# JinPLu/VeloxSeg

Hardware: AMD Instinct MI355X
Metric: training patches/s on 128^3 2-mod volumes (fwd+loss+bwd+allreduce+AdamW) (higher is better)
Workload: dtype f32

## Files before the change

### include/veloxseg_hip.h

```cpp
#ifndef VELOXSEG_HIP_H
#define VELOXSEG_HIP_H

#ifdef __cplusplus
extern "C" {
#endif

#define VX_ABI_VERSION 1

int vx_abi_version(void);
const char* vx_last_error(void);

int vx_conv3d_fwd(const float* x, const float* x2, int C1, const float* w, const float* bias, float* y,
                  int B, int Cin, int Di, int Hi, int Wi, int Cout, int K, int S, int P, int G, int ps, void* stream);
int vx_conv3d_bwd_data(const float* dy, const float* w, const float* bias_like, float* dx, float* dx2, int C1,
                       int B, int Cin, int Di, int Hi, int Wi, int Cout, int K, int S, int P, int G, int ps,
                       int accumulate, void* stream);
int vx_conv3d_bwd_weight(const float* x, const float* x2, int C1, const float* dy, float* dw, float* db,
                         int B, int Cin, int Di, int Hi, int Wi, int Cout, int K, int S, int P, int G, int ps, void* stream);

int vx_conv3d_bwd_weight_tiled(const float* x, const float* x2, int C1, const float* dy, float* dw, float* db,
                               int B, int Cin, int Di, int Hi, int Wi, int Cout, int K, int S, int P, int G, int ps, void* stream);
int vx_down_wgrad_ws_floats(int B, int Cin, int Di, int Hi, int Wi, int Cout);
int vx_down_wgrad_mfma(const float* x, const float* dy, float* dw, float* db, float* ws, long ws_floats,
                       int B, int Cin, int Di, int Hi, int Wi, int Cout, void* stream);
// ... 32 lines not shown
                   int B, int Cin, int Cout, long V, void* stream);
int vx_pw_conv_set_v4(int on);
int vx_pw_conv_bwd_data(const float* dy, const float* w, float* dx, float* dx2, int C1,
                        int B, int Cin, int Cout, long V, int accumulate, void* stream);
int vx_pw_conv_bwd_weight(const float* x, const float* x2, int C1, const float* dy, float* dw, float* db,
                          int B, int Cin, int Cout, long V, void* stream);
int vx_pw_conv_fwd_h(const void* x, const float* w, const float* bias, float* y, int B, int Cin, int Cout, long V, int x_h16, void* stream);
int vx_pw_conv_bwd_weight_h(const void* x, const float* dy, float* dw, float* db, int B, int Cin, int Cout, long V, int x_h16, void* stream);

int vx_pw_conv_mfma(const float* src, const float* src2, int S1, const float* w, int transpose_w, const float* bias,
                    float* dst, float* dst2, int D1, int B, int Mch, int Kch, int Cin_of_w, long V, int accumulate, void* stream);
int vx_pw_conv_bwd_fused(const float* dy, const float* w, const float* x, const float* x2, int C1, float* dx, float* dx2, float* dw, float* db,
                         int B, int Cin, int Cout, long V, int accumulate, void* stream);
int vx_pw_conv_bwd_fused_big(const float* dy, const float* w, const float* x, const float* x2, int C1, float* dx, float* dx2, float* dw, float* db,
                             int B, int Cin, int Cout, long V, int accumulate, void* stream);
int vx_pw_conv_gelu_fwd(const float* x, const float* w, const float* bias, float* a, float* h, int B, int Cin, int Cout, long V, int mfma,
                        const void* seed_ptr, unsigned long long dstream, float p, void* stream);
int vx_pw_conv_gelu_bwd_data(const float* dy, const float* w, const float* a, float* da, int B, int Cin, int Cout, long V, int mfma,
                             const void* seed_ptr, unsigned long long dstream, float p, void* stream);
int vx_pw_conv_res_fwd(const float* x, const float* w, const float* bias, const float* res, float* out, int B, int Cin, int Cout, long V, int mfma,
                       float alpha, const void* seed_ptr, unsigned long long dstream, float p, void* stream);
int vx_pw_mfma_set_wide(int on);

int vx_mlp_supported(int C, int R, long V);
int vx_mlp_bwd_nparts(int B, int C, long V);
int vx_mlp_fwd(const float* x, int norm, const double* part, int nparts, float* stats, const float* gamma, const float* beta,
               const float* w1, const float* b1, const float* w2, const float* b2, float* out, int B, int C, int R, long V, float eps,
               const void* seed_ptr, unsigned long long site1, float p1, unsigned long long site2, float p2, void* stream);
int vx_mlp_bwd(const float* x, int norm, const float* stats, const float* gamma, const float* beta, const float* w1, const float* b1,
               const float* w2, const float* dout, float* dx, float* part_out, float* dgamma, float* dbeta, float* dw1, float* db1,
               float* dw2, float* db2, int B, int C, int R, long V, float eps, const void* seed_ptr, unsigned long long site1, float p1,
               unsigned long long site2, float p2, void* stream);
int vx_jlc_ntiles(int B, int C, int G, int D, int H, int W);
int vx_jlc_nchunks(long BC, long V);
int vx_jlc_conv_fwd(const float* x, const float* w1, const float* w3, const float* w5, const float* b1, const float* b3, const float* b5,
                    float* y1, float* y3, float* y5, double* part, int B, int C, int G, int D, int H, int W, void* stream);
int vx_jlc_mid_fwd(const float* x, const float* y1, const float* y3, const float* y5, const double* part_y, int nty, float* stats_y, float* o,
                   double* part_o, long BC, long V, float eps, void* stream);
int vx_jlc_mid_bwd(const float* dout, const float* dn, const float* part_dn, int npd, const float* o, const float* stats_o, const float* y1,
                   const float* y3, const float* y5, const float* stats_y, float* d_o, float* part_t, long BC, long V, void* stream);
int vx_jlc_gk(const float* d_o, const float* y1, const float* y3, const float* y5, const float* stats_y, const float* part_t, float* g1, float* g3,
              float* g5, long BC, long V, void* stream);
int vx_jlc_conv_bwd(const float* g1, const float* g3, const float* g5, const float* w1, const float* w3, const float* w5, const float* d_o,
                    float* dx, int B, int C, int G, int D, int H, int W, void* stream);
int vx_jlc_mid_fwd_h(const float* x, const void* y1, const void* y3, const void* y5, const double* part_y, int nty, float* stats_y, void* o,
                     double* part_o, long BC, long V, float eps, int h16, void* stream);
int vx_jlc_mid_bwd_h(const float* dout, const void* dn, const float* part_dn, int npd, const void* o, const float* stats_o, const void* y1,
                     const void* y3, const void* y5, const float* stats_y, void* d_o, float* part_t, long BC, long V, int h16, void* stream);
int vx_jlc_gk_h(const void* d_o, const void* y1, const void* y3, const void* y5, const float* stats_y, const float* part_t, void* g1, void* g3,
                void* g5, long BC, long V, int h16, void* stream);
int vx_mlp_fwd_h(const void* x, int norm, const double* part, int nparts, float* stats, const float* gamma, const float* beta,
                 const float* w1, const float* b1, const float* w2, const float* b2, float* out, int B, int C, int R, long V, float eps,
                 const void* seed_ptr, unsigned long long site1, float p1, unsigned long long site2, float p2, int h16, void* stream);
int vx_mlp_bwd_h(const void* x, int norm, const float* stats, const float* gamma, const float* beta, const float* w1, const float* b1,
                 const float* w2, const float* dout, void* dx, float* part_out, float* dgamma, float* dbeta, float* dw1, float* db1,
                 float* dw2, float* db2, int B, int C, int R, long V, float eps, const void* seed_ptr, unsigned long long site1, float p1,
                 unsigned long long site2, float p2, int h16, void* stream);

int vx_jlc_tz_ok(int C, int G, int D, int H, int W);
int vx_jlc_tz_ntiles(int C, int G, int D, int H, int W);
int vx_jlc_tz_img_floats(int C, int G);
int vx_jlc_tz_set_pieces(int ns);
int vx_jlc_tz_set_min_voxels(long v);
int vx_jlc_tz_pieces(void);
int vx_jlc_tz_set_debug(int mask);
int vx_jlc_tz_prep(const float* w1, const float* w3, const float* w5, float* img, int C, int G, void* stream);
int vx_jlc_tz_fwd(const float* x, const float* img, const float* b1, const float* b3, const float* b5, float* y1, float* y3, float* y5, double* part,
                  int B, int C, int G, int D, int H, int W, void* stream);
int vx_jlc_tz_bwd(const float* g1, const float* g3, const float* g5, const float* img, const float* w1, const float* d_o, float* dx,
                  int B, int C, int G, int D, int H, int W, void* stream);
int vx_jlc_cl_ok(int C, int G, int D, int H, int W);
int vx_jlc_cl_ntiles(int C, int G, int D, int H, int W);
int vx_jlc_cl_img_floats(int C, int G);
int vx_jlc_cl_set_enabled(int on);
int vx_jlc_cl_prep(const float* w1, const float* w3, const float* w5, float* img, int C, int G, void* stream);
int vx_jlc_cl_fwd(const float* x, const float* img, const float* b1, const float* b3, const float* b5, float* y1, float* y3, float* y5, double* part,
                  int B, int C, int G, int D, int H, int W, void* stream);
int vx_jlc_cl_bwd(const float* g1, const float* g3, const float* g5, const float* img, const float* d_o, float* dx, int B, int C, int G, int D, int H, int W,
                  void* stream);
int vx_jlc_wgrad_tz_ok(int C, int G, int D, int H, int W);
int vx_jlc_wgrad_tz_set_min_voxels(long v);
int vx_jlc_wgrad_tz_set_blocks(int n);
int vx_jlc_wgrad_tz_set_spec(int on);
int vx_jlc_wgrad_tz_set_f16(int on);
int vx_jlc_wgrad_tz(const float* x, const float* g1, const float* g3, const float* g5, float* dw1, float* dw3, float* dw5, int B, int C, int G, int D, int H, int W,
                    void* stream);
int vx_jlc_tz_img_floats_ns(int C, int G, int pieces);
int vx_jlc_tz_prep_ns(const float* w1, const float* w3, const float* w5, float* img, int C, int G, int pieces, void* stream);
int vx_jlc_tz_fwd_ns(const float* x, const float* img, const float* b1, const float* b3, const float* b5, float* y1, float* y3, float* y5, double* part,
                     int B, int C, int G, int D, int H, int W, int pieces, void* stream);
int vx_jlc_tz_bwd_ns(const float* g1, const float* g3, const float* g5, const float* img, const float* w1, const float* d_o, float* dx,
                     int B, int C, int G, int D, int H, int W, int pieces, void* stream);
int vx_jlc_wgrad_tz_ns(const float* x, const float* g1, const float* g3, const float* g5, float* dw1, float* dw3, float* dw5, int B, int C, int G, int D, int H, int W,
                       int pieces, void* stream);
int vx_jlc_tz_fwd_h(const float* x, const float* img, const float* b1, const float* b3, const float* b5, void* y1, void* y3, void* y5, double* part,
                    int B, int C, int G, int D, int H, int W, int pieces, int h16, void* stream);
int vx_jlc_tz_bwd_h(const void* g1, const void* g3, const void* g5, const float* img, const float* w1, const void* d_o, float* dx,
                    int B, int C, int G, int D, int H, int W, int pieces, int h16, void* stream);
int vx_jlc_wgrad_tz_h(const float* x, const void* g1, const void* g3, const void* g5, float* dw1, float* dw3, float* dw5, int B, int C, int G, int D, int H, int W,
                      int pieces, int h16, void* stream);

int vx_in_stats(const float* x, float* stats, double* part_ws, long BC, long V, float eps, void* stream);
int vx_in_apply_fwd(const float* y0, const float* y1, const float* y2, const float* s0, const float* s1, const float* s2,
                    int nk, int act, const float* res, float* out, long BC, long V, void* stream);
int vx_in_bwd(const float* dout, const float* y, const float* stats, int act, float* m_ws, double* part_ws, float* dy, long BC, long V, void* stream);
int vx_in_row_max(void);
int vx_in_row_fwd(const float* y0, const float* y1, const float* y2, float* s0, float* s1, float* s2, int nk, int act, const float* res,
                  float* out, long BC, long V, float eps, void* stream);
int vx_in_row_bwd(const float* dout, const float* y0, const float* y1, const float* y2, const float* s0, const float* s1, const float* s2,
                  int nk, int act, float* d0, float* d1, float* d2, long BC, long V, void* stream);
int vx_in_bwd_db(const float* dout, const float* y, const float* stats, int act, float* m_ws, double* part_ws, float* dy, long BC, long V, float* db, int C, void* stream);
int vx_in_fwd_split(const float* y0, const float* y1, const float* y2, float* s0, float* s1, float* s2, double* part_ws,
                    int nk, int act, const float* res, float* out, long BC, long V, float eps, void* stream);
int vx_in_bwd_split(const float* dout, const float* y0, const float* y1, const float* y2, const float* s0, const float* s1, const float* s2,
                    double* part_ws, int nk, int act, float* dy0, float* dy1, float* dy2, const float* add0, long BC, long V, void* stream);
int vx_in_row_bwd_add(const float* dout, const float* y0, const float* stats0, int act, const float* add0, float* d0, long BC, long V, void* stream);
int vx_in_row_bwd_db(const float* dout, const float* y0, const float* y1, const float* y2, const float* s0, const float* s1, const float* s2,
                     int nk, int act, float* d0, float* d1, float* d2, float* db0, float* db1, float* db2, int C, long BC, long V, void* stream);

int vx_ln_cf_fwd(const float* x, const float* gamma, const float* beta, float* out, int B, int C, long V, float eps, void* stream);
int vx_ln_cf_bwd(const float* x, const float* gamma, const float* dout, float* dx, float* dgamma, float* dbeta, float* ws,
                 int B, int C, long V, float eps, void* stream);
int vx_ln_cf_bwd_add(const float* x, const float* gamma, const float* dout, const float* add, float* dx, float* dgamma, float* dbeta, float* ws,
                     int B, int C, long V, float eps, void* stream);
int vx_ln_cf_bwd_data(const float* x, const float* gamma, const float* dout, const float* add, float* dx, float* ws, int B, int C, long V, float eps, void* stream);
int vx_ln_cf_bwd_param(const float* x, const float* dout, const float* ws, float* dgamma, float* dbeta, int B, int C, long V, void* stream);

int vx_gelu_drop_fwd(const float* a, float* h, long n, const void* seed_ptr, unsigned long long dstream, float p, void* stream);
int vx_gelu_drop_bwd(const float* dh, const float* a, float* da, long n, const void* seed_ptr, unsigned long long dstream, float p, void* stream);
int vx_axpy_drop_fwd(const float* x, const float* z, float* out, float alpha, long n, const void* seed_ptr, unsigned long long dstream, float p, void* stream);
int vx_axpy_drop_bwd(const float* dout, float* dx, float* dz, float alpha, long n, const void* seed_ptr, unsigned long long dstream, float p, void* stream);
int vx_add(const float* a, const float* b, const float* c, float* out, long n, void* stream);
int vx_add_many(const float* const* a, const float* const* b, const float* const* c, float* const* out, const long* n, int count, void* stream);
int vx_channel_sum(const float* dy, float* db, int B, int C, long V, void* stream);
int vx_space_to_depth2(const float* x, float* out, int B, int C, int Dc, int Hc, int Wc, int inverse, void* stream);
int vx_patchify(const float* x, float* out, int B, int C, int d, int h, int w, int K, void* stream);
int vx_patchify_bs(const float* x, long batch_stride, float* out, int B, int C, int d, int h, int w, int K, void* stream);
int vx_patchify_bs_h(const float* x, long batch_stride, void* out, int B, int C, int d, int h, int w, int K, int out_h16, void* stream);
int vx_patch_embed_ok(int Cin, int Cout, int Do, int Ho, int Wo, int K);
int vx_patch_embed_fwd(const float* x, long batch_stride, const float* w, const float* bias, float* y, int B, int Cin, int Cout, int Do, int Ho, int Wo, void* stream);
int vx_patch_embed_bwd_weight(const float* x, long batch_stride, const float* dy, float* dw, float* db, int B, int Cin, int Cout, int Do, int Ho, int Wo, void* stream);

typedef struct VxPwaPlan {
    int grid[3];
    int n[3];
    int heads, nb;
    int small[4][3];
    int nwin[4][3];
    int woff[4];
    int Ntot;
    int l;
} VxPwaPlan;

int vx_pwa_gather_fwd(const float* src, float* tok, const VxPwaPlan* plan, int c, int m, int M, int B, void* stream);
int vx_pwa_gather_bwd(const float* src, const float* dtok, float* dsrc, const VxPwaPlan* plan, int c, int m, int M, int B, void* stream);
int vx_pwa_gather_all_fwd(const float* const* srcs, float* tq, float* tk, float* tv, int* iq, int* ik, int* iv,
                          const VxPwaPlan* plan, int cq, int cv, int M, int B, void* stream);
int vx_pwa_gather_all_bwd(const float* dtq, const float* dtk, const float* dtv, const int* iq, const int* ik, const int* iv, float* const* dsrcs,
                          const VxPwaPlan* plan, int cq, int cv, int M, int B, void* stream);
int vx_pwa_scatter_fwd(const float* tok, float* out, const VxPwaPlan* plan, int c, int m, int M, int B, void* stream);
int vx_pwa_scatter_bwd(const float* dout, float* dtok, const VxPwaPlan* plan, int c, int m, int M, int B, void* stream);
int vx_pwa_scatter_fwd_all(const float* tok, float* const* outs, const VxPwaPlan* plan, int c, int M, int B, void* stream);
int vx_pwa_scatter_bwd_all(const float* const* douts, float* dtok, const VxPwaPlan* plan, int c, int M, int B, void* stream);
int vx_pwa_scatter_bwd_all_w(const float* const* douts, float* dtok, const VxPwaPlan* plan, int c, int M, int B, void* stream);
int vx_pwa_scatter_bwd_all_wz(const float* const* douts, float* dtok, const VxPwaPlan* plan, int c, int M, int B, float* extra_zero, long extra_floats, void* stream);
int vx_pwa_attn_set_fused_bwd(int on);
int vx_pwa_scatter_set_ident(int on);
// ... 174 lines not shown
```

### veloxseg_amd/csrc/jlc_mfma.hip

```cpp
#include "vx_common.h"
#include <type_traits>
#include "../../include/veloxseg_hip.h"

typedef __bf16 tz_bf8 __attribute__((ext_vector_type(8)));
typedef float tz_f4 __attribute__((ext_vector_type(4)));

struct TzGeo {
    int HD, HH;
    int Sd, Sc, Sp;
    int nrows;
    unsigned mHH, mHD;
    int qd0, nq;
    unsigned mNQ;
};

struct VxTz {
    const void* src[3];
    const uint4* img;
    const float* esc;
    const float* bias[3];
    const void* res;
    const float* w1;
    void* out[3];
    double* part;
// ... 740 lines not shown
        if (s + 1 < NS) { a0 -= tz_lo(lo); a1 -= tz_hi(lo); a2 -= tz_lo(hi); a3 -= tz_hi(hi); }
    }
}

#define WG_NPF 6
struct WgDesc { const char* b; int l, f; };
template <bool H16 = false>
__device__ __forceinline__ WgDesc wg_desc(const VxWgT& p, int it, int sg, int cob, int cib, int h0) {
    WgDesc r;
    r.b = (const char*)p.x; r.l = 0; r.f = 0;
    const int nqx = p.XR / 4, rows = p.TH + 4;
    const int nx = p.nb * 4 * rows * nqx;
    const int chan = p.D * p.H * p.W;
    if (it < nx) {
        const int qd = it % nqx; int t = it / nqx;
        const int row = t % rows; t /= rows;
        const int ci = t & 3, s = t >> 2;
        const int b = sg * p.nb + s, ih = h0 - 2 + row, iw = 4 * qd - 4;
        const bool ok = b < p.B && (unsigned)ih < (unsigned)p.H && (unsigned)iw < (unsigned)p.W;
        r.f = 4 | (ok ? 8 : 0);
        r.b = (const char*)(p.x + (ok ? (long)(b * p.C + cib + ci) * chan + ih * p.W + iw : 0));
        r.l = ((s * 4 + ci) * rows + row) * p.XR + 4 * qd;
        return r;
    }
    it -= nx;
    const int nqg = p.WS / 4;
    const int ng = p.nb * 4 * p.TH * nqg;
    const int kind = it / ng;
    if (kind > 2) return r;
    it -= kind * ng;
    const int qd = it % nqg; int t = it / nqg;
    const int row = t % p.TH; t /= p.TH;
    const int co = t & 3, s = t >> 2;
    const int b = sg * p.nb + s, ih = h0 + row, iw = 4 * qd;
    const bool ok = b < p.B && ih < p.H && iw < p.W;
    r.f = (kind + 1) | 4 | (ok ? 8 : 0);
    r.b = (const char*)(kind == 0 ? p.g5 : kind == 1 ? p.g3 : p.g1) + (H16 ? 2L : 4L) * (ok ? (long)(b * p.C + cob + co) * chan + ih * p.W + iw : 0);
    r.l = p.GB + ((s * 4 + co) * (p.TH + 1) + row) * p.WS + 4 * qd;
    return r;
}
__device__ __forceinline__ int wg_dk(int k) { return (0x18 >> (2 * k)) & 3; }
template <bool SP> __device__ __forceinline__ int wg_s5(const VxWgT&, int pl) { return (pl + 60) % (SP ? 6 : 5); }
template <bool SP> __device__ __forceinline__ int wg_s3(const VxWgT&, int pl) { return (SP ? 6 : 5) + (pl + 60) % (SP ? 4 : 3); }
template <bool SP> __device__ __forceinline__ int wg_s1(const VxWgT&, int pl) { return SP ? 10 + ((pl + 60) & 1) : 8; }
template <bool SP> __device__ __forceinline__ int wg_xo(const VxWgT& p, int dx) { return SP ? ((dx + 60) & 1) * p.XP : 0; }
template <bool H16 = false>
__device__ __forceinline__ void wg_prefetch(float4 (&pf)[WG_NPF], const WgDesc (&ds)[WG_NPF], const VxWgT& p, int dx, int dg0, int dg1) {
    const long HW = (long)p.H * p.W;
#pragma unroll
    for (int u = 0; u < WG_NPF; ++u) {
        const int k = ds[u].f & 3;
        const int pl = dx + wg_dk(k);
        const bool on = (ds[u].f & 8) && pl >= (k == 0 ? 0 : dg0) && pl < (k == 0 ? p.D : dg1);
        typedef const __attribute__((address_space(1))) tz_f4* wg_gptr;
        if constexpr (H16) {
            typedef unsigned int wg_u2 __attribute__((ext_vector_type(2)));
            typedef const __attribute__((address_space(1))) wg_u2* wg_gptr2;
            const bool isx = k == 0;
            const unsigned long long ga = (unsigned long long)ds[u].b + (isx ? 4ull : 2ull) * (unsigned long long)(on ? (long)pl * HW : 0);
            float4 r;
            if (isx) { const tz_f4 v = *(wg_gptr)ga; r = make_float4(v[0], v[1], v[2], v[3]); }
            else { const wg_u2 v = *(wg_gptr2)ga; r = make_float4(vx_bf16_lo(v[0]), vx_bf16_hi(v[0]), vx_bf16_lo(v[1]), vx_bf16_hi(v[1])); }
            pf[u] = on ? r : make_float4(0.f, 0.f, 0.f, 0.f);
        } else {
        const unsigned long long ga = (unsigned long long)ds[u].b + 4ull * (unsigned long long)(on ? (long)pl * HW : 0);
        const tz_f4 v = *(wg_gptr)ga;
        pf[u] = on ? make_float4(v[0], v[1], v[2], v[3]) : make_float4(0.f, 0.f, 0.f, 0.f);
        }
    }
}
template <int NS, bool SP = false>
__device__ __forceinline__ void wg_commit(const float4 (&pf)[WG_NPF], const WgDesc (&ds)[WG_NPF], unsigned char* lds, const VxWgT& p, int dx, int dg0, int dg1) {
    const int l5 = wg_s5<SP>(p, dx + 2) * p.GP, l3 = wg_s3<SP>(p, dx + 1) * p.GP, l1 = wg_s1<SP>(p, dx) * p.GP, lx = wg_xo<SP>(p, dx);
#pragma unroll
    for (int u = 0; u < WG_NPF; ++u) {
        const int k = ds[u].f & 3;
        const int pl = dx + wg_dk(k);
        const bool on = (ds[u].f & 4) && pl >= (k == 0 ? 0 : dg0) && pl < (k == 0 ? p.D : dg1);
        const int lo = k == 0 ? lx : k == 1 ? l5 : k == 2 ? l3 : l1;
        if (on) wg_split_store<NS>(pf[u], lds, (long)ds[u].l + lo, p.SP);
    }
}

__device__ __forceinline__ void wg_commit16(const float4 (&pf)[WG_NPF], const WgDesc (&ds)[WG_NPF], unsigned char* lds, const VxWgT& p, int dx, int dg0, int dg1,
                                            float* __restrict__ mtab, int* __restrict__ etab) {
    const int s5 = wg_s5<false>(p, dx + 2), s3 = wg_s3<false>(p, dx + 1), s1_ = wg_s1<false>(p, dx);
    const int l5 = s5 * p.GP, l3 = s3 * p.GP, l1 = s1_ * p.GP;
    float mk[4] = {0.f, 0.f, 0.f, 0.f};
    bool on_[WG_NPF];
#pragma unroll
    for (int u = 0; u < WG_NPF; ++u) {
        const int k = ds[u].f & 3;
        const int pl = dx + wg_dk(k);
        on_[u] = (ds[u].f & 4) && pl >= (k == 0 ? 0 : dg0) && pl < (k == 0 ? p.D : dg1);
        const float m_ = on_[u] ? fmaxf(fmaxf(fabsf(pf[u].x), fabsf(pf[u].y)), fmaxf(fabsf(pf[u].z), fabsf(pf[u].w))) : 0.0f;
#pragma unroll
        for (int kk = 0; kk < 4; ++kk) mk[kk] = fmaxf(mk[kk], k == kk ? m_ : 0.0f);
    }
#pragma unroll
    for (int kk = 0; kk < 4; ++kk) mk[kk] = vx_wave_max(mk[kk]);
    if ((threadIdx.x & 63) == 0) {
#pragma unroll
        for (int kk = 0; kk < 4; ++kk) mtab[(threadIdx.x >> 6) * 4 + kk] = mk[kk];
    }
    __syncthreads();
    int ek[4];
#pragma unroll
    for (int kk = 0; kk < 4; ++kk) ek[kk] = tz_exp16(fmaxf(fmaxf(mtab[kk], mtab[4 + kk]), fmaxf(mtab[8 + kk], mtab[12 + kk])));
    if (threadIdx.x == 0) {
        etab[0] = ek[0];
        etab[1 + s5] = ek[1]; etab[1 + s3] = ek[2]; etab[1 + s1_] = ek[3];
    }
#pragma unroll
    for (int u = 0; u < WG_NPF; ++u) {
        if (!on_[u]) continue;
        const int k = ds[u].f & 3;
        const int lo = k == 0 ? 0 : k == 1 ? l5 : k == 2 ? l3 : l1;
        const float sc = ldexpf(1.0f, k == 0 ? ek[0] : k == 1 ? ek[1] : k == 2 ? ek[2] : ek[3]);
        const float a0 = pf[u].x * sc, a1 = pf[u].y * sc, a2 = pf[u].z * sc, a3 = pf[u].w * sc;
        const uint32_t lo0 = tz_pack16(a0, a1), hi0 = tz_pack16(a2, a3);
        const uint32_t lo1 = tz_pack16(a0 - tz_lo16(lo0), a1 - tz_hi16(lo0)), hi1 = tz_pack16(a2 - tz_lo16(hi0), a3 - tz_hi16(hi0));
        const long e0 = (long)ds[u].l + lo;
        *reinterpret_cast<uint2*>(lds + 2 * e0) = make_uint2(lo0, hi0);
        *reinterpret_cast<uint2*>(lds + 2 * ((long)p.SP + e0)) = make_uint2(lo1, hi1);
    }
}

template <int NS>
__device__ __forceinline__ void wg_read_a(uint4 (&a)[NS], const unsigned char* lds, const VxWgT& p, int slot, int arow_base, int local, int th_lane) {
    const int j = threadIdx.x & 3;
    const int r = local + j;
    const int rr = (unsigned)r < (unsigned)th_lane ? r : p.TH;
#pragma unroll
    for (int s = 0; s < NS; ++s)
        a[s] = *reinterpret_cast<const uint4*>(lds + 2 * ((long)s * p.SP + p.GB + (long)slot * p.GP + (long)arow_base + (long)rr * p.WS));
}

template <int NS, bool F16 = false>
__device__ __forceinline__ void wg_mfma6(tz_f4& acc, const uint4 (&a)[NS], const uint4 (&b)[NS]) {
    constexpr int NP = NS == 3 ? 6 : NS == 2 ? 3 : 1;
    constexpr int PW[6] = {1, 2, 0, 1, 0, 0}, PA[6] = {1, 0, 2, 0, 1, 0};
    constexpr int PW2[3] = {1, 0, 0}, PA2[3] = {0, 1, 0};
#pragma unroll
    for (int pr = 0; pr < NP; ++pr) {
        const int sa = NS == 3 ? PW[pr] : NS == 2 ? PW2[pr] : 0, sb = NS == 3 ? PA[pr] : NS == 2 ? PA2[pr] : 0;
        if constexpr (F16) acc = __builtin_amdgcn_mfma_f32_16x16x32_f16(__builtin_bit_cast(tz_h8, a[sa]), __builtin_bit_cast(tz_h8, b[sb]), acc, 0, 0, 0);
        else acc = __builtin_amdgcn_mfma_f32_16x16x32_bf16(__builtin_bit_cast(tz_bf8, a[sa]), __builtin_bit_cast(tz_bf8, b[sb]), acc, 0, 0, 0);
    }
}

__device__ __forceinline__ uint4 wg_shift(const uint32_t (&w)[8], int o) {
    const int d = o >> 1;
    if ((o & 1) == 0) return make_uint4(w[d], w[d + 1], w[d + 2], w[d + 3]);
    return make_uint4(__builtin_amdgcn_alignbit(w[d + 1], w[d], 16), __builtin_amdgcn_alignbit(w[d + 2], w[d + 1], 16), __builtin_amdgcn_alignbit(w[d + 3], w[d + 2], 16),
                      __builtin_amdgcn_alignbit(w[d + 4], w[d + 3], 16));
}

template <int NS, bool DBG, bool F16 = false, bool SPEC = false, bool H16 = false>
__global__ void __launch_bounds__(SPEC ? 512 : 256, SPEC ? 1 : 2) vx_jlc_wg_k(VxWgT p_) {
    const VxWgT& p = p_;
    const int dbg = DBG ? p_.dbg : 0;
    extern __shared__ __attribute__((aligned(16))) unsigned char wg_lds[];
    const int lane = threadIdx.x & 63;
    const int wave = __builtin_amdgcn_readfirstlane((int)(threadIdx.x >> 6));
    const int r16 = lane & 15, q = lane >> 4;
    int bid = blockIdx.x;
    const int dc = bid % p.nDc; bid /= p.nDc;
    const int ht = bid % p.nHt; bid /= p.nHt;
    const int MT = p.CG >> 2;
    const int ih = bid % MT; bid /= MT;
    const int ch = bid % MT; bid /= MT;
    const int g = bid % p.G;
    const int sg = bid / p.G;
    const int h0 = ht * p.TH;
    const int dg0 = dc * p.DC, dg1 = min(p.D, dg0 + p.DC);
    const int cob = g * p.CG + ch * 4, cib = g * p.CG + ih * 4;

    constexpr int nslot = SPEC ? 12 : 9;
    for (int it = threadIdx.x; it < nslot * p.nb * 4 * (p.WS / 2) * NS; it += blockDim.x) {
        int r = it;
        const int e2 = r % (p.WS / 2); r /= (p.WS / 2);
        const int sc = r % (p.nb * 4); r /= (p.nb * 4);
        const int slot = r % nslot, s = r / nslot;
        *reinterpret_cast<uint32_t*>(wg_lds + 2 * ((long)s * p.SP + p.GB + (long)slot * p.GP + ((long)sc * (p.TH + 1) + p.TH) * p.WS + 2 * e2)) = 0u;
    }
    const int smp_ = (8 * q) / p.WS;
    const bool nosmp = smp_ >= p.nb;
    const int smp = nosmp ? 0 : smp_, wq = nosmp ? 0 : 8 * q - smp_ * p.WS;
    const int arow_base = ((smp * 4 + (r16 >> 2)) * (p.TH + 1)) * p.WS + wq;
    const int brow_base = ((smp * 4 + (r16 >> 2)) * (p.TH + 4) + (r16 & 3)) * p.XR + wq;
    const int th_lane = nosmp ? 0 : p.TH;

    tz_f4 acc[20];
    float* mtab = reinterpret_cast<float*>(wg_lds + 2 * (long)NS * p.SP);
    int* etab = reinterpret_cast<int*>(mtab + 16);
    int ecur[5] = {0, 0, 0, 0, 0};
    const bool producer = SPEC && wave >= 4;
    if (SPEC && producer) {
        float4 pf[WG_NPF];
        WgDesc ds[WG_NPF];
#pragma unroll
        for (int u = 0; u < WG_NPF; ++u) ds[u] = wg_desc<H16>(p, (int)(threadIdx.x & 255) + u * 256, sg, cob, cib, h0);
        wg_prefetch<H16>(pf, ds, p, dg0 - 2, dg0, dg1);
        __syncthreads();
        wg_commit<NS, true>(pf, ds, wg_lds, p, dg0 - 2, dg0, dg1);
        wg_prefetch<H16>(pf, ds, p, dg0 - 1, dg0, dg1);
        __syncthreads();
        for (int dx = dg0 - 2; dx <= dg1 + 1; ++dx) {
            if (dx + 1 <= dg1 + 1) {
                wg_commit<NS, true>(pf, ds, wg_lds, p, dx + 1, dg0, dg1);
                if (dx + 2 <= dg1 + 1) wg_prefetch<H16>(pf, ds, p, dx + 2, dg0, dg1);
            }
            __syncthreads();
        }
    } else {
#pragma unroll
    for (int t = 0; t < 20; ++t) acc[t] = (tz_f4){0.f, 0.f, 0.f, 0.f};
    float4 pf[WG_NPF];
    WgDesc ds[WG_NPF];
    if constexpr (!SPEC) {
#pragma unroll
        for (int u = 0; u < WG_NPF; ++u) ds[u] = wg_desc<H16>(p, (int)threadIdx.x + u * 256, sg, cob, cib, h0);
        wg_prefetch<H16>(pf, ds, p, dg0 - 2, dg0, dg1);
    } else {
        __syncthreads();
        __syncthreads();
    }
    for (int dx = dg0 - 2; dx <= dg1 + 1; ++dx) {
        if constexpr (SPEC) {
            if ((unsigned)dx >= (unsigned)p.D) { __syncthreads(); continue; }
        } else {
        __syncthreads();
        if constexpr (F16) wg_commit16(pf, ds, wg_lds, p, dx, dg0, dg1, mtab, etab);
        else if (!(dbg & 1)) wg_commit<NS>(pf, ds, wg_lds, p, dx, dg0, dg1);
        __syncthreads();
        if (dx + 1 <= dg1 + 1 && !(dbg & 1)) wg_prefetch<H16>(pf, ds, p, dx + 1, dg0, dg1);
        if (dbg & 2) continue;
        if ((unsigned)dx >= (unsigned)p.D) continue;
        }
        const bool k3w = wave < 3;
        const int kd0 = k3w ? wave : 3, kd1 = k3w ? wave : 4;
        const int pl0 = dx - kd0 + 2, pl1 = k3w ? dx - kd1 + 1 : dx - kd1 + 2;
        const bool ok0 = pl0 >= dg0 && pl0 < dg1, ok1 = pl1 >= dg0 && pl1 < dg1, okc = wave == 0 && dx >= dg0 && dx < dg1;
        const int so0 = wg_s5<SPEC>(p, pl0), so1 = k3w ? wg_s3<SPEC>(p, pl1) : wg_s5<SPEC>(p, pl1);
        const int xo8 = wg_xo<SPEC>(p, dx) >> 3;
        if constexpr (F16) {
            const int e_x = __builtin_amdgcn_readfirstlane(etab[0]);
            auto bring = [&](int which, int slot, int lo, int n_) {
                const int ep = e_x + __builtin_amdgcn_readfirstlane(etab[1 + slot]);
                if (ep == ecur[which]) return;
                const int dd = ep - ecur[which];
                const float f = ldexpf(1.0f, dd > 120 ? 120 : (dd < -120 ? -120 : dd));
#pragma unroll
                for (int t = 0; t < 20; ++t)
                    if (t >= lo && t < lo + n_ && !(which == 1 && k3w && (t == 13 || t == 14 || t == 18 || t == 19))) acc[t] *= f;
                ecur[which] = ep;
            };
            if (ok0) bring(0, so0, 0, 10);
            if (ok1) bring(1, so1, 10, 10);
            if (okc) {
                const int ep = e_x + __builtin_amdgcn_readfirstlane(etab[1 + wg_s1<SPEC>(p, dx)]);
                if (ep != ecur[4]) {
                    const int dd = ep - ecur[4];
                    acc[13] *= ldexpf(1.0f, dd > 120 ? 120 : (dd < -120 ? -120 : dd));
                    ecur[4] = ep;
                }
            }
        }
        for (int xb = 0; xb < p.nXB; ++xb) {
            uint32_t w[NS][8];
#pragma unroll
            for (int s = 0; s < NS; ++s) {
                const int eo = ((s * (p.SP >> 3) + xo8 + (brow_base >> 3) + 4 * xb * (p.XR >> 3)) << 3);
                const uint4* bp = reinterpret_cast<const uint4*>(wg_lds + 2 * (long)eo);
                const uint4 lo = bp[0], hi = bp[1];
                w[s][0] = lo.x; w[s][1] = lo.y; w[s][2] = lo.z; w[s][3] = lo.w; w[s][4] = hi.x; w[s][5] = hi.y; w[s][6] = hi.z; w[s][7] = hi.w;
            }
            uint4 sh[5][NS];
#pragma unroll
            for (int k = 0; k < 5; ++k)
#pragma unroll
                for (int s = 0; s < NS; ++s) sh[k][s] = wg_shift(w[s], k + 2);
            uint4 a[NS];
#pragma unroll
            for (int u = 0; u < 4; ++u) {
                const int sl = u >> 1, typ = u & 1;
                const bool k3 = sl == 1 && k3w;
                if (!(sl ? ok1 : ok0)) continue;
                const int local = 4 * xb - (typ ? 4 : 0) - (k3 ? 1 : 0);
                if (local + 3 < 0 || local >= p.TH) continue;
                if (!(dbg & 16)) wg_read_a<NS>(a, wg_lds, p, sl ? so1 : so0, arow_base, local, th_lane);
#pragma unroll
                for (int k = 0; k < 5; ++k) {
                    if (k >= 3 && k3) continue;
                    if (!(dbg & 8)) wg_mfma6<NS, F16>(acc[5 * u + k], a, sh[sl ? (k + 1) % 5 : k]);
                }
            }
            if (okc) {
                wg_read_a<NS>(a, wg_lds, p, wg_s1<SPEC>(p, dx), arow_base, 4 * xb - 2, th_lane);
                wg_mfma6<NS, F16>(acc[13], a, sh[2]);
            }
        }
        if constexpr (SPEC) __syncthreads();
    }
    }
    if (dbg & 4) return;
    float* tl = reinterpret_cast<float*>(wg_lds);
    if constexpr (F16) {
        const float f0 = ldexpf(1.0f, -ecur[0]), f1 = ldexpf(1.0f, -ecur[1]), f13 = ldexpf(1.0f, -ecur[4]);
#pragma unroll
        for (int t = 0; t < 20; ++t) {
            if (t < 10) acc[t] *= f0;
            else if (wave < 3 && (t == 13 || t == 14 || t == 18 || t == 19)) { if (t == 13) acc[t] *= f13; }
            else acc[t] *= f1;
        }
    }
#pragma unroll
    for (int sl = 0; sl < 2; ++sl) {
        __syncthreads();
        if (!SPEC || wave < 4) {
#pragma unroll
        for (int t = 0; t < 10; ++t)
            *reinterpret_cast<float4*>(tl + (((wave * 10 + t) * 16 + r16) * 16 + 4 * q)) = make_float4(acc[sl * 10 + t][0], acc[sl * 10 + t][1], acc[sl * 10 + t][2], acc[sl * 10 + t][3]);
        }
        __syncthreads();
        const int n5 = sl == 0 ? 1600 : 400, n3 = sl == 0 ? 0 : 432;
        for (int it = threadIdx.x; it < n5 + n3; it += blockDim.x) {
            const bool k3 = it >= n5;
            const int o = k3 ? it - n5 : it;
            const int K = k3 ? 3 : 5, per = k3 ? 27 : (sl == 0 ? 100 : 25);
            const int pair = o / per, r = o - pair * per;
            const int kdl = r / (K * K), r2 = r - kdl * K * K;
            const int kh = r2 / K, kw = r2 - kh * K;
            const int kd = k3 ? kdl : (sl == 0 ? kdl : 4);
            const int wv = k3 ? kd : (kd < 3 ? kd : 3);
            const int co = pair >> 2, ci = pair & 3;
            const int kt = (!k3 && sl == 1) ? (kw + 4) % 5 : kw;
            float v = 0.0f;
#pragma unroll
            for (int typ = 0; typ < 2; ++typ) {
                const float* T = tl + ((wv * 10 + typ * 5 + kt) * 16) * 16;
                const int d = kh - (typ ? 4 : 0);
#pragma unroll
                for (int jj = 0; jj < 4; ++jj) {
                    const int i = jj + d;
                    if (i >= 0 && i < 4) v += T[(ci * 4 + i) * 16 + co * 4 + jj];
                }
            }
            float* dst = k3 ? p.dw3 : p.dw5;
            const int K3 = K * K * K;
            if (dst) atomicAdd(dst + ((long)(cob + co) * p.CG + ih * 4 + ci) * K3 + (kd * K + kh) * K + kw, v);
        }
        if (sl == 1 && p.dw1) {
            for (int pair = threadIdx.x; pair < 16; pair += blockDim.x) {
                const int co = pair >> 2, ci = pair & 3;
                const float* T = tl + ((0 * 10 + 3) * 16) * 16;
                float v = 0.0f;
#pragma unroll
                for (int jj = 0; jj < 4; ++jj) v += T[(ci * 4 + jj) * 16 + co * 4 + jj];
                atomicAdd(p.dw1 + (long)(cob + co) * p.CG + ih * 4 + ci, v);
            }
        }
    }
}

static int g_wg_blocks = 0;
extern "C" int vx_jlc_wgrad_tz_set_blocks(int n) { g_wg_blocks = n > 0 ? n : 0; return 0; }
static int g_wg_spec = 1;
extern "C" int vx_jlc_wgrad_tz_set_spec(int on) { g_wg_spec = on ? 1 : 0; return 0; }
static bool wg_spec_on() { return g_wg_spec == 1; }
static int wg_plan(VxWgT& p, size_t& shm, int B, int C, int G, int D, int H, int W, int NS, bool spec = false) {
    if (B <= 0 || C <= 0 || G <= 0 || C % G || D <= 0 || H <= 0 || W <= 0 || (W & 3) || (H & 3) || W > 32) return -1;
    const int CG = C / G;
    if (CG != 4 && CG != 8 && CG != 16) return -1;
    p.B = B; p.C = C; p.G = G; p.D = D; p.H = H; p.W = W; p.CG = CG;
    p.WS = (W + 7) / 8 * 8;
    p.nb = 32 / p.WS;
    p.nsg = vx_cdiv(B, p.nb);
    p.TH = H % 8 == 0 ? 8 : 4;
    p.nHt = H / p.TH;
    p.nXB = p.TH / 4 + 1;
    p.XR = p.WS + 8;
    p.XP = p.nb * 4 * (p.TH + 4) * p.XR;
    p.GP = p.nb * 4 * (p.TH + 1) * p.WS;
    p.XB = spec ? 2 : 1; p.R5 = spec ? 6 : 5; p.R3 = spec ? 4 : 3; p.R1 = spec ? 2 : 1;
    p.GB = p.XB * p.XP;
    p.SP = p.GB + (p.R5 + p.R3 + p.R1) * p.GP;
    const int MT = CG / 4;
    const long base_blocks = (long)p.nsg * G * MT * MT * p.nHt;
    const int target = g_wg_blocks > 0 ? g_wg_blocks : (spec ? 128 : 256);
    int nchunks = (int)((target + base_blocks - 1) / base_blocks);
    constexpr int min_dc = 2;
    if (nchunks > D / min_dc) nchunks = D / min_dc;
    if (nchunks < 1) nchunks = 1;
    p.DC = vx_cdiv(D, nchunks);
    p.nDc = vx_cdiv(D, p.DC);
    if ((long)p.nb * 4 * (p.TH + 4) * (p.XR / 4) + 3L * p.nb * 4 * p.TH * (p.WS / 4) > (long)WG_NPF * 256) return -1;
    shm = (size_t)NS * p.SP * 2 + 128;
    if (shm < 4 * 10 * 256 * sizeof(float)) shm = 4 * 10 * 256 * sizeof(float);
    if (shm > 150 * 1024) return -1;
    return 0;
}

static long g_wg_min_v = 0;
static int g_wg_f16 = 0;
extern "C" int vx_jlc_wgrad_tz_set_f16(int on) { g_wg_f16 = on ? 1 : 0; return 0; }
extern "C" int vx_jlc_wgrad_tz_set_min_voxels(long v) { g_wg_min_v = v < 0 ? 0 : v; return 0; }
extern "C" int vx_jlc_wgrad_tz_ok(int C, int G, int D, int H, int W) {
    VxWgT p = {};
    size_t shm;
    if ((long)D * H * W < g_wg_min_v) return 0;
    return wg_plan(p, shm, 1, C, G, D, H, W, tz_pieces() == 22 ? 3 : tz_pieces()) == 0 ? 1 : 0;
}

extern "C" int vx_jlc_wgrad_tz(const float* x, const float* g1, const float* g3, const float* g5, float* dw1, float* dw3, float* dw5, int B, int C, int G, int D, int H, int W,
                               void* stream) {
    VX_REQUIRE(x && g1 && g3 && g5, "vx_jlc_wgrad_tz: null pointer");
    VxWgT p = {};
    size_t shm;
    const bool f16 = tz_pieces() == 22 && g_wg_f16 == 1;
    const int NS = f16 ? 2 : (tz_pieces() == 22 ? 3 : tz_pieces());
    VX_REQUIRE(!t_tz_h16 || NS == 1, "vx_jlc_wgrad_tz: 16-bit g_k need plain bf16 operands (pieces = 1, the bf16 mode)");
    bool spec = !f16 && NS == 3 && (g_tz_dbg >> 4) == 0 && wg_spec_on();
    if (spec) { VxWgT q = {}; size_t sh2; spec = wg_plan(q, sh2, B, C, G, D, H, W, NS, true) == 0; }
    VX_REQUIRE(wg_plan(p, shm, B, C, G, D, H, W, NS, spec) == 0, "vx_jlc_wgrad_tz: unsupported shape C=%d G=%d %dx%dx%d", C, G, D, H, W);
    p.x = x; p.g1 = g1; p.g3 = g3; p.g5 = g5; p.dw1 = dw1; p.dw3 = dw3; p.dw5 = dw5; p.dbg = g_tz_dbg >> 4;
    const int MT = p.CG / 4;
    const dim3 grid((unsigned)((long)p.nsg * G * MT * MT * p.nHt * p.nDc));
    hipStream_t st = (hipStream_t)stream;
#define WG_LAUNCH(ns)                                                                                                                                      \
    do {                                                                                                                                                   \
        static bool attr = false;                                                                                                                          \
        if (!attr) {                                                                                                                                       \
            VX_REQUIRE(hipFuncSetAttribute((const void*)vx_jlc_wg_k<ns, false>, hipFuncAttributeMaxDynamicSharedMemorySize, 160 * 1024) == hipSuccess &&           \
                       hipFuncSetAttribute((const void*)vx_jlc_wg_k<ns, true>, hipFuncAttributeMaxDynamicSharedMemorySize, 160 * 1024) == hipSuccess, "vx_jlc_wgrad_tz: LDS attribute"); \
            attr = true;                                                                                                                                   \
        }                                                                                                                                                  \
        if (p.dbg) vx_jlc_wg_k<ns, true><<<grid, dim3(256), shm, st>>>(p);                                                                                 \
        else vx_jlc_wg_k<ns, false><<<grid, dim3(256), shm, st>>>(p);                                                                                      \
    } while (0)
    if (spec) {
        static bool attrs = false;
        if (!attrs) { VX_REQUIRE(hipFuncSetAttribute((const void*)vx_jlc_wg_k<3, false, false, true>, hipFuncAttributeMaxDynamicSharedMemorySize, 160 * 1024) == hipSuccess, "vx_jlc_wgrad_tz: LDS attribute"); attrs = true; }
        vx_jlc_wg_k<3, false, false, true><<<grid, dim3(512), shm, st>>>(p);
    } else if (f16) {
        static bool attr16 = false;
        if (!attr16) { VX_REQUIRE(hipFuncSetAttribute((const void*)vx_jlc_wg_k<2, false, true>, hipFuncAttributeMaxDynamicSharedMemorySize, 160 * 1024) == hipSuccess, "vx_jlc_wgrad_tz: LDS attribute"); attr16 = true; }
        vx_jlc_wg_k<2, false, true><<<grid, dim3(256), shm, st>>>(p);
    } else if (NS == 3) WG_LAUNCH(3); else if (NS == 2) WG_LAUNCH(2);
    else if (t_tz_h16) {
        static bool attrh = false;
        if (!attrh) { VX_REQUIRE(hipFuncSetAttribute((const void*)vx_jlc_wg_k<1, false, false, false, true>, hipFuncAttributeMaxDynamicSharedMemorySize, 160 * 1024) == hipSuccess, "vx_jlc_wgrad_tz: LDS attribute"); attrh = true; }
        vx_jlc_wg_k<1, false, false, false, true><<<grid, dim3(256), shm, st>>>(p);
    } else WG_LAUNCH(1);
#undef WG_LAUNCH
    VX_LAUNCH_CHECK("vx_jlc_wgrad_tz");
    return 0;
}

extern "C" int vx_jlc_tz_img_floats_ns(int C, int G, int pieces) {
    if (!tz_pieces_valid(pieces)) return -1;
    TzPiecesScope sc(pieces);
    return vx_jlc_tz_img_floats(C, G);
}
extern "C" int vx_jlc_tz_prep_ns(const float* w1, const float* w3, const float* w5, float* img, int C, int G, int pieces, void* stream) {
    VX_REQUIRE(tz_pieces_valid(pieces), "vx_jlc_tz_prep_ns: pieces %d", pieces);
    TzPiecesScope sc(pieces);
    return vx_jlc_tz_prep(w1, w3, w5, img, C, G, stream);
}
extern "C" int vx_jlc_tz_fwd_ns(const float* x, const float* img, const float* b1, const float* b3, const float* b5, float* y1, float* y3, float* y5, double* part,
                                int B, int C, int G, int D, int H, int W, int pieces, void* stream) {
    VX_REQUIRE(tz_pieces_valid(pieces), "vx_jlc_tz_fwd_ns: pieces %d", pieces);
    TzPiecesScope sc(pieces);
    return vx_jlc_tz_fwd(x, img, b1, b3, b5, y1, y3, y5, part, B, C, G, D, H, W, stream);
}
extern "C" int vx_jlc_tz_bwd_ns(const float* g1, const float* g3, const float* g5, const float* img, const float* w1, const float* d_o, float* dx,
                                int B, int C, int G, int D, int H, int W, int pieces, void* stream) {
    VX_REQUIRE(tz_pieces_valid(pieces), "vx_jlc_tz_bwd_ns: pieces %d", pieces);
    TzPiecesScope sc(pieces);
    return vx_jlc_tz_bwd(g1, g3, g5, img, w1, d_o, dx, B, C, G, D, H, W, stream);
}
extern "C" int vx_jlc_tz_fwd_h(const float* x, const float* img, const float* b1, const float* b3, const float* b5, void* y1, void* y3, void* y5, double* part,
                               int B, int C, int G, int D, int H, int W, int pieces, int h16, void* stream) {
    VX_REQUIRE(tz_pieces_valid(pieces), "vx_jlc_tz_fwd_h: pieces %d", pieces);
    TzPiecesScope sc(pieces);
    TzH16Scope hs(h16 ? 1 : 0);
    return vx_jlc_tz_fwd(x, img, b1, b3, b5, (float*)y1, (float*)y3, (float*)y5, part, B, C, G, D, H, W, stream);
}
extern "C" int vx_jlc_tz_bwd_h(const void* g1, const void* g3, const void* g5, const float* img, const float* w1, const void* d_o, float* dx,
                               int B, int C, int G, int D, int H, int W, int pieces, int h16, void* stream) {
    VX_REQUIRE(tz_pieces_valid(pieces), "vx_jlc_tz_bwd_h: pieces %d", pieces);
    TzPiecesScope sc(pieces);
    TzH16Scope hs(h16 ? 1 : 0);
    return vx_jlc_tz_bwd((const float*)g1, (const float*)g3, (const float*)g5, img, w1, (const float*)d_o, dx, B, C, G, D, H, W, stream);
}
extern "C" int vx_jlc_wgrad_tz_h(const float* x, const void* g1, const void* g3, const void* g5, float* dw1, float* dw3, float* dw5, int B, int C, int G, int D, int H, int W,
                                 int pieces, int h16, void* stream) {
    VX_REQUIRE(tz_pieces_valid(pieces), "vx_jlc_wgrad_tz_h: pieces %d", pieces);
    TzPiecesScope sc(pieces);
    TzH16Scope hs(h16 ? 1 : 0);
    return vx_jlc_wgrad_tz(x, (const float*)g1, (const float*)g3, (const float*)g5, dw1, dw3, dw5, B, C, G, D, H, W, stream);
}
extern "C" int vx_jlc_wgrad_tz_ns(const float* x, const float* g1, const float* g3, const float* g5, float* dw1, float* dw3, float* dw5, int B, int C, int G, int D, int H, int W,
                                  int pieces, void* stream) {
    VX_REQUIRE(tz_pieces_valid(pieces), "vx_jlc_wgrad_tz_ns: pieces %d", pieces);
    TzPiecesScope sc(pieces);
    return vx_jlc_wgrad_tz(x, g1, g3, g5, dw1, dw3, dw5, B, C, G, D, H, W, stream);
}
```

Measured before the change: 1088.

## Enable warp-specialized producer/consumer pipeline for f16 two-piece JLC weight-gradient kernel

Adds a warp-specialized variant of the f16 (two-piece scaled fp16 split) JLC weight-gradient kernel. Producer waves compute per-slab max exponents and commit scaled halves into double-buffered exponent tables, while consumer waves run the MFMA accumulation. It makes this f16 spec path the default when pieces==22 and the shape fits, replacing the three-piece bf16 spec path. It also adds a zero-slab sentinel so rescaling is skipped for all-zero slabs, lowers the block target and pads LDS to limit occupancy. The aim is fewer MFMA pieces per product with the conversion overlapped with compute, at the cost of fp16 range and precision in gradient accumulation and extra synchronisation.

```diff
diff --git a/include/veloxseg_hip.h b/include/veloxseg_hip.h
--- a/include/veloxseg_hip.h
+++ b/include/veloxseg_hip.h
@@ -138,7 +138,7 @@
 int vx_jlc_wgrad_tz_set_min_voxels(long v);
 int vx_jlc_wgrad_tz_set_blocks(int n);
 int vx_jlc_wgrad_tz_set_spec(int on);
-int vx_jlc_wgrad_tz_set_f16(int on);
+int vx_jlc_wgrad_tz_set_f16(int mode);
 int vx_jlc_wgrad_tz(const float* x, const float* g1, const float* g3, const float* g5, float* dw1, float* dw3, float* dw5, int B, int C, int G, int D, int H, int W,
                     void* stream);
 int vx_jlc_tz_img_floats_ns(int C, int G, int pieces);
diff --git a/veloxseg_amd/csrc/jlc_mfma.hip b/veloxseg_amd/csrc/jlc_mfma.hip
--- a/veloxseg_amd/csrc/jlc_mfma.hip
+++ b/veloxseg_amd/csrc/jlc_mfma.hip
@@ -846,6 +846,7 @@
     }
 }
 
+#define WG_EZ (1 << 20)
 __device__ __forceinline__ void wg_commit16(const float4 (&pf)[WG_NPF], const WgDesc (&ds)[WG_NPF], unsigned char* lds, const VxWgT& p, int dx, int dg0, int dg1,
                                             float* __restrict__ mtab, int* __restrict__ etab) {
     const int s5 = wg_s5<false>(p, dx + 2), s3 = wg_s3<false>(p, dx + 1), s1_ = wg_s1<false>(p, dx);
@@ -868,18 +869,73 @@
         for (int kk = 0; kk < 4; ++kk) mtab[(threadIdx.x >> 6) * 4 + kk] = mk[kk];
     }
     __syncthreads();
-    int ek[4];
-#pragma unroll
-    for (int kk = 0; kk < 4; ++kk) ek[kk] = tz_exp16(fmaxf(fmaxf(mtab[kk], mtab[4 + kk]), fmaxf(mtab[8 + kk], mtab[12 + kk])));
+    int ek[4], et[4];
+#pragma unroll
+    for (int kk = 0; kk < 4; ++kk) {
+        const float m_ = fmaxf(fmaxf(mtab[kk], mtab[4 + kk]), fmaxf(mtab[8 + kk], mtab[12 + kk]));
+        ek[kk] = tz_exp16(m_);
+        et[kk] = m_ == 0.0f ? WG_EZ : ek[kk];
+    }
     if (threadIdx.x == 0) {
-        etab[0] = ek[0];
-        etab[1 + s5] = ek[1]; etab[1 + s3] = ek[2]; etab[1 + s1_] = ek[3];
+        etab[0] = et[0];
+        etab[1 + s5] = et[1]; etab[1 + s3] = et[2]; etab[1 + s1_] = et[3];
     }
 #pragma unroll
     for (int u = 0; u < WG_NPF; ++u) {
         if (!on_[u]) continue;
         const int k = ds[u].f & 3;
         const int lo = k == 0 ? 0 : k == 1 ? l5 : k == 2 ? l3 : l1;
+        const float sc = ldexpf(1.0f, k == 0 ? ek[0] : k == 1 ? ek[1] : k == 2 ? ek[2] : ek[3]);
+        const float a0 = pf[u].x * sc, a1 = pf[u].y * sc, a2 = pf[u].z * sc, a3 = pf[u].w * sc;
+        const uint32_t lo0 = tz_pack16(a0, a1), hi0 = tz_pack16(a2, a3);
+        const uint32_t lo1 = tz_pack16(a0 - tz_lo16(lo0), a1 - tz_hi16(lo0)), hi1 = tz_pack16(a2 - tz_lo16(hi0), a3 - tz_hi16(hi0));
+        const long e0 = (long)ds[u].l + lo;
+        *reinterpret_cast<uint2*>(lds + 2 * e0) = make_uint2(lo0, hi0);
+        *reinterpret_cast<uint2*>(lds + 2 * ((long)p.SP + e0)) = make_uint2(lo1, hi1);
+    }
+}
+
+__device__ __forceinline__ void wg_max16(const float4 (&pf)[WG_NPF], const WgDesc (&ds)[WG_NPF], const VxWgT& p, int s, int dg0, int dg1, float* __restrict__ mtab) {
+    float mk[4] = {0.f, 0.f, 0.f, 0.f};
+#pragma unroll
+    for (int u = 0; u < WG_NPF; ++u) {
+        const int k = ds[u].f & 3;
+        const int pl = s + wg_dk(k);
+        const bool on = (ds[u].f & 4) && pl >= (k == 0 ? 0 : dg0) && pl < (k == 0 ? p.D : dg1);
+        const float m_ = on ? fmaxf(fmaxf(fabsf(pf[u].x), fabsf(pf[u].y)), fmaxf(fabsf(pf[u].z), fabsf(pf[u].w))) : 0.0f;
+#pragma unroll
+        for (int kk = 0; kk < 4; ++kk) mk[kk] = fmaxf(mk[kk], k == kk ? m_ : 0.0f);
+    }
+#pragma unroll
+    for (int kk = 0; kk < 4; ++kk) mk[kk] = vx_wave_max(mk[kk]);
+    if ((threadIdx.x & 63) == 0) {
+#pragma unroll
+        for (int kk = 0; kk < 4; ++kk) mtab[((s + 60) & 1) * 16 + ((threadIdx.x >> 6) & 3) * 4 + kk] = mk[kk];
+    }
+}
+__device__ __forceinline__ void wg_commit16s(const float4 (&pf)[WG_NPF], const WgDesc (&ds)[WG_NPF], unsigned char* lds, const VxWgT& p, int s, int dg0, int dg1,
+                                             const float* __restrict__ mtab, int* __restrict__ etab) {
+    const int s5 = wg_s5<true>(p, s + 2), s3 = wg_s3<true>(p, s + 1), s1_ = wg_s1<true>(p, s);
+    const int l5 = s5 * p.GP, l3 = s3 * p.GP, l1 = s1_ * p.GP, lx = wg_xo<true>(p, s);
+    const float* mt = mtab + ((s + 60) & 1) * 16;
+    int ek[4], et[4];
+#pragma unroll
+    for (int kk = 0; kk < 4; ++kk) {
+        const float m_ = fmaxf(fmaxf(mt[kk], mt[4 + kk]), fmaxf(mt[8 + kk], mt[12 + kk]));
+        ek[kk] = tz_exp16(m_);
+        et[kk] = m_ == 0.0f ? WG_EZ : ek[kk];
+    }
+    if ((threadIdx.x & 255) == 0) {
+        etab[(s + 60) & 1] = et[0];
+        etab[2 + s5] = et[1]; etab[2 + s3] = et[2]; etab[2 + s1_] = et[3];
+    }
+#pragma unroll
+    for (int u = 0; u < WG_NPF; ++u) {
+        const int k = ds[u].f & 3;
+        const int pl = s + wg_dk(k);
+        const bool on = (ds[u].f & 4) && pl >= (k == 0 ? 0 : dg0) && pl < (k == 0 ? p.D : dg1);
+        if (!on) continue;
+        const int lo = k == 0 ? lx : k == 1 ? l5 : k == 2 ? l3 : l1;
         const float sc = ldexpf(1.0f, k == 0 ? ek[0] : k == 1 ? ek[1] : k == 2 ? ek[2] : ek[3]);
         const float a0 = pf[u].x * sc, a1 = pf[u].y * sc, a2 = pf[u].z * sc, a3 = pf[u].w * sc;
         const uint32_t lo0 = tz_pack16(a0, a1), hi0 = tz_pack16(a2, a3);
@@ -957,7 +1013,8 @@
 
     tz_f4 acc[20];
     float* mtab = reinterpret_cast<float*>(wg_lds + 2 * (long)NS * p.SP);
-    int* etab = reinterpret_cast<int*>(mtab + 16);
+    int* etab = reinterpret_cast<int*>(mtab + (SPEC ? 32 : 16));
+    constexpr int EB = SPEC ? 2 : 1;
     int ecur[5] = {0, 0, 0, 0, 0};
     const bool producer = SPEC && wave >= 4;
     if (SPEC && producer) {
@@ -965,6 +1022,31 @@
         WgDesc ds[WG_NPF];
 #pragma unroll
         for (int u = 0; u < WG_NPF; ++u) ds[u] = wg_desc<H16>(p, (int)(threadIdx.x & 255) + u * 256, sg, cob, cib, h0);
+        if constexpr (F16) {
+            float4 pg[WG_NPF];
+            const int last = dg1 + 1;
+            auto stage = [&](const float4 (&cur)[WG_NPF], float4 (&nxt)[WG_NPF], int s) {
+                if (s > last || (dbg & 1)) return;
+                if (s + 1 <= last) wg_prefetch<H16>(nxt, ds, p, s + 1, dg0, dg1);
+                wg_commit16s(cur, ds, wg_lds, p, s, dg0, dg1, mtab, etab);
+                if (s + 1 <= last) wg_max16(nxt, ds, p, s + 1, dg0, dg1, mtab);
+            };
+            if (DBG && threadIdx.x - 256 < 14) etab[threadIdx.x - 256] = 0;
+            if (!(dbg & 1)) {
+                wg_prefetch<H16>(pf, ds, p, dg0 - 2, dg0, dg1);
+                wg_max16(pf, ds, p, dg0 - 2, dg0, dg1, mtab);
+            }
+            __syncthreads();
+            stage(pf, pg, dg0 - 2);
+            __syncthreads();
+            for (int dx = dg0 - 2; dx <= last; dx += 2) {
+                stage(pg, pf, dx + 1);
+                __syncthreads();
+                if (dx + 1 > last) break;
+                stage(pf, pg, dx + 2);
+                __syncthreads();
+            }
+        } else {
         wg_prefetch<H16>(pf, ds, p, dg0 - 2, dg0, dg1);
         __syncthreads();
         wg_commit<NS, true>(pf, ds, wg_lds, p, dg0 - 2, dg0, dg1);
@@ -977,6 +1059,7 @@
             }
             __syncthreads();
         }
+        }
     } else {
 #pragma unroll
     for (int t = 0; t < 20; ++t) acc[t] = (tz_f4){0.f, 0.f, 0.f, 0.f};
@@ -992,7 +1075,7 @@
     }
     for (int dx = dg0 - 2; dx <= dg1 + 1; ++dx) {
         if constexpr (SPEC) {
-            if ((unsigned)dx >= (unsigned)p.D) { __syncthreads(); continue; }
+            if ((unsigned)dx >= (unsigned)p.D || (dbg & 2)) { __syncthreads(); continue; }
         } else {
         __syncthreads();
         if constexpr (F16) wg_commit16(pf, ds, wg_lds, p, dx, dg0, dg1, mtab, etab);
@@ -1009,10 +1092,11 @@
         const int so0 = wg_s5<SPEC>(p, pl0), so1 = k3w ? wg_s3<SPEC>(p, pl1) : wg_s5<SPEC>(p, pl1);
         const int xo8 = wg_xo<SPEC>(p, dx) >> 3;
         if constexpr (F16) {
-            const int e_x = __builtin_amdgcn_readfirstlane(etab[0]);
+            const int e_x = __builtin_amdgcn_readfirstlane(etab[SPEC ? (dx + 60) & 1 : 0]);
             auto bring = [&](int which, int slot, int lo, int n_) {
-                const int ep = e_x + __builtin_amdgcn_readfirstlane(etab[1 + slot]);
-                if (ep == ecur[which]) return;
+                const int e_g = __builtin_amdgcn_readfirstlane(etab[EB + slot]);
+                const int ep = e_x + e_g;
+                if (e_x == WG_EZ || e_g == WG_EZ || ep == ecur[which]) return;
                 const int dd = ep - ecur[which];
                 const float f = ldexpf(1.0f, dd > 120 ? 120 : (dd < -120 ? -120 : dd));
 #pragma unroll
@@ -1023,8 +1107,9 @@
             if (ok0) bring(0, so0, 0, 10);
             if (ok1) bring(1, so1, 10, 10);
             if (okc) {
-                const int ep = e_x + __builtin_amdgcn_readfirstlane(etab[1 + wg_s1<SPEC>(p, dx)]);
-                if (ep != ecur[4]) {
+                const int e_g = __builtin_amdgcn_readfirstlane(etab[EB + wg_s1<SPEC>(p, dx)]);
+                const int ep = e_x + e_g;
+                if (e_x != WG_EZ && e_g != WG_EZ && ep != ecur[4]) {
                     const int dd = ep - ecur[4];
                     acc[13] *= ldexpf(1.0f, dd > 120 ? 120 : (dd < -120 ? -120 : dd));
                     ecur[4] = ep;
@@ -1133,7 +1218,7 @@
 static int g_wg_spec = 1;
 extern "C" int vx_jlc_wgrad_tz_set_spec(int on) { g_wg_spec = on ? 1 : 0; return 0; }
 static bool wg_spec_on() { return g_wg_spec == 1; }
-static int wg_plan(VxWgT& p, size_t& shm, int B, int C, int G, int D, int H, int W, int NS, bool spec = false) {
+static int wg_plan(VxWgT& p, size_t& shm, int B, int C, int G, int D, int H, int W, int NS, bool spec = false, bool f16 = false) {
     if (B <= 0 || C <= 0 || G <= 0 || C % G || D <= 0 || H <= 0 || W <= 0 || (W & 3) || (H & 3) || W > 32) return -1;
     const int CG = C / G;
     if (CG != 4 && CG != 8 && CG != 16) return -1;
@@ -1152,7 +1237,7 @@
     p.SP = p.GB + (p.R5 + p.R3 + p.R1) * p.GP;
     const int MT = CG / 4;
     const long base_blocks = (long)p.nsg * G * MT * MT * p.nHt;
-    const int target = g_wg_blocks > 0 ? g_wg_blocks : (spec ? 128 : 256);
+    const int target = g_wg_blocks > 0 ? g_wg_blocks : (spec ? (f16 ? 96 : 128) : 256);
     int nchunks = (int)((target + base_blocks - 1) / base_blocks);
     constexpr int min_dc = 2;
     if (nchunks > D / min_dc) nchunks = D / min_dc;
@@ -1160,15 +1245,17 @@
     p.DC = vx_cdiv(D, nchunks);
     p.nDc = vx_cdiv(D, p.DC);
     if ((long)p.nb * 4 * (p.TH + 4) * (p.XR / 4) + 3L * p.nb * 4 * p.TH * (p.WS / 4) > (long)WG_NPF * 256) return -1;
-    shm = (size_t)NS * p.SP * 2 + 128;
+    shm = (size_t)NS * p.SP * 2 + (spec ? 256 : 128);
     if (shm < 4 * 10 * 256 * sizeof(float)) shm = 4 * 10 * 256 * sizeof(float);
     if (shm > 150 * 1024) return -1;
+    if (spec && f16 && shm < 81 * 1024) shm = 81 * 1024;
     return 0;
 }
 
 static long g_wg_min_v = 0;
+#define WG_F16_DEFAULT 1
 static int g_wg_f16 = 0;
-extern "C" int vx_jlc_wgrad_tz_set_f16(int on) { g_wg_f16 = on ? 1 : 0; return 0; }
+extern "C" int vx_jlc_wgrad_tz_set_f16(int mode) { g_wg_f16 = mode == 1 || mode == 2 ? mode : 0; return 0; }
 extern "C" int vx_jlc_wgrad_tz_set_min_voxels(long v) { g_wg_min_v = v < 0 ? 0 : v; return 0; }
 extern "C" int vx_jlc_wgrad_tz_ok(int C, int G, int D, int H, int W) {
     VxWgT p = {};
@@ -1182,12 +1269,13 @@
     VX_REQUIRE(x && g1 && g3 && g5, "vx_jlc_wgrad_tz: null pointer");
     VxWgT p = {};
     size_t shm;
-    const bool f16 = tz_pieces() == 22 && g_wg_f16 == 1;
+    const bool spec_fits16 = [&] { VxWgT q = {}; size_t sh2; return wg_plan(q, sh2, B, C, G, D, H, W, 2, true, true) == 0; }();
+    const bool f16 = tz_pieces() == 22 && (g_wg_f16 == 1 || (g_wg_f16 == 0 && WG_F16_DEFAULT && wg_spec_on() && spec_fits16));
     const int NS = f16 ? 2 : (tz_pieces() == 22 ? 3 : tz_pieces());
     VX_REQUIRE(!t_tz_h16 || NS == 1, "vx_jlc_wgrad_tz: 16-bit g_k need plain bf16 operands (pieces = 1, the bf16 mode)");
-    bool spec = !f16 && NS == 3 && (g_tz_dbg >> 4) == 0 && wg_spec_on();
-    if (spec) { VxWgT q = {}; size_t sh2; spec = wg_plan(q, sh2, B, C, G, D, H, W, NS, true) == 0; }
-    VX_REQUIRE(wg_plan(p, shm, B, C, G, D, H, W, NS, spec) == 0, "vx_jlc_wgrad_tz: unsupported shape C=%d G=%d %dx%dx%d", C, G, D, H, W);
+    bool spec = wg_spec_on() && (f16 ? spec_fits16 : NS == 3 && (g_tz_dbg >> 4) == 0);
+    if (spec && !f16) { VxWgT q = {}; size_t sh2; spec = wg_plan(q, sh2, B, C, G, D, H, W, NS, true) == 0; }
+    VX_REQUIRE(wg_plan(p, shm, B, C, G, D, H, W, NS, spec, f16) == 0, "vx_jlc_wgrad_tz: unsupported shape C=%d G=%d %dx%dx%d", C, G, D, H, W);
     p.x = x; p.g1 = g1; p.g3 = g3; p.g5 = g5; p.dw1 = dw1; p.dw3 = dw3; p.dw5 = dw5; p.dbg = g_tz_dbg >> 4;
     const int MT = p.CG / 4;
     const dim3 grid((unsigned)((long)p.nsg * G * MT * MT * p.nHt * p.nDc));
@@ -1203,7 +1291,16 @@
         if (p.dbg) vx_jlc_wg_k<ns, true><<<grid, dim3(256), shm, st>>>(p);                                                                                 \
         else vx_jlc_wg_k<ns, false><<<grid, dim3(256), shm, st>>>(p);                                                                                      \
     } while (0)
-    if (spec) {
+    if (spec && f16) {
+        static bool attrs16 = false;
+        if (!attrs16) {
+            VX_REQUIRE(hipFuncSetAttribute((const void*)vx_jlc_wg_k<2, false, true, true>, hipFuncAttributeMaxDynamicSharedMemorySize, 160 * 1024) == hipSuccess &&
+                       hipFuncSetAttribute((const void*)vx_jlc_wg_k<2, true, true, true>, hipFuncAttributeMaxDynamicSharedMemorySize, 160 * 1024) == hipSuccess, "vx_jlc_wgrad_tz: LDS attribute");
+            attrs16 = true;
+        }
+        if (p.dbg) vx_jlc_wg_k<2, true, true, true><<<grid, dim3(512), shm, st>>>(p);
+        else vx_jlc_wg_k<2, false, true, true><<<grid, dim3(512), shm, st>>>(p);
+    } else if (spec) {
         static bool attrs = false;
         if (!attrs) { VX_REQUIRE(hipFuncSetAttribute((const void*)vx_jlc_wg_k<3, false, false, true>, hipFuncAttributeMaxDynamicSharedMemorySize, 160 * 1024) == hipSuccess, "vx_jlc_wgrad_tz: LDS attribute"); attrs = true; }
         vx_jlc_wg_k<3, false, false, true><<<grid, dim3(512), shm, st>>>(p);
```

After: 1093, median of 6. Within noise of the previous version (+0.5%).
